# arkworks-rs/accumulation

Hardware: AMD Instinct MI355X
Metric: MSM throughput (point-scalar pairs/sec) at 2^20 Pallas (higher is better)
Workload: dtype u32; 1 GPU; 2^20-pair pallas MSM per GPU (north_star size; scalars uniform in [0, r), G_i = k_i*G), key resident + precomputed window multiples; pairs_per_gpu=1048576, curve=pallas, precomputed_key=True, parallelism=point-sharded x1, window_bits=20, pipeline=bucket-per-lane (k_prep_local_t + k_accum_bpl; skewed scalars re-run chunked), window_widths=9 x 20 + 4 x 19 bits = 256 (MsmGeom::n_narrow), msms_in_flight=3, full=False

## Files before the change

### accumulation_amd/csrc/api_pipeline.inc

```

#define HIP_TRY(expr)                                                                                  \
  do {                                                                                                 \
    hipError_t _e = (expr);                                                                            \
    if (_e != hipSuccess) {                                                                            \
      fprintf(stderr, "[amsm] HIP error %s (%d) at %s:%d: %s\n", hipGetErrorName(_e), (int)_e, __FILE__, \
              __LINE__, #expr);                                                                        \
      return _e == hipErrorOutOfMemory ? AMSM_E_OOM : AMSM_E_HIP;                                      \
    }                                                                                                  \
  } while (0)

#define TRY(expr)            \
  do {                       \
    int _s = (expr);         \
    if (_s != AMSM_OK) return _s; \
  } while (0)

int ensure(DevBuf& b, size_t bytes) {
  if (b.bytes >= bytes && b.p) return AMSM_OK;
  if (b.p) HIP_TRY(hipFree(b.p));
  b.p = nullptr;
  b.bytes = 0;
  size_t want = bytes + bytes / 8 + 256;
  HIP_TRY(hipMalloc(&b.p, want));
  b.bytes = want;
// ... 176 lines not shown
#define AMSM_DBG(name)                                    \
  do {                                                    \
    if (amsm_debug()) {                                   \
      fprintf(stderr, "[amsm] %s ...", name);             \
      hipError_t e_ = hipDeviceSynchronize();             \
      fprintf(stderr, " %s\n", hipGetErrorString(e_));    \
    }                                                     \
  } while (0)

int prep_fork(amsm_ctx* ctx) {
  HIP_TRY(hipEventRecord(ctx->fork, ctx->stream));
  HIP_TRY(hipStreamWaitEvent(ctx->s_prep, ctx->fork, 0));
  return AMSM_OK;
}

template <class Fq>
int bases_alt(amsm_ctx* ctx, const amsm_bases* b, const amsm_bases** out);

inline size_t bpl_min_pairs(const amsm_bases*) { return msel::P2(18) + 1; }

inline bool bpl_geom(amsm_ctx* ctx, const amsm_bases* bases, size_t base_off, size_t n, int group_shift, int c_plain, MsmGeom* out) {
  MsmGeom g;
  if (make_geom(ctx, bases, base_off, n, &g, group_shift, c_plain) != AMSM_OK) return false;
  if (g.groups == 1u && g.precomp) {
    u32 b = 1;
    while ((1ull << b) < n) b++;
    unsigned long long abs_max = (unsigned long long)g.base_off + n - 1ull + (unsigned long long)(g.W - 1u) * g.table_stride;
    unsigned long long rel_max = ((unsigned long long)(g.W - 1u) << b) | ((1ull << b) - 1ull);
    if (rel_max < abs_max) g.idx_rel_bits = b;
  }
  g.bpl = 1;
  {
    unsigned long long raw_max = 0;
    (void)top_window_shift_curve(ctx->curve, (int)g.c, (int)g.W, (int)g.n_narrow, &raw_max);
    unsigned long long top_reach = std::min<unsigned long long>(g.nb, raw_max << (g.top_shift + (g.n_narrow ? 1u : 0u)));
    top_reach = std::max<unsigned long long>(1024ull, top_reach);
    const unsigned long long per_win = ((unsigned long long)n * 1024ull + g.nb - 1) / g.nb;
    const unsigned long long per_top = ((unsigned long long)n * 1024ull + top_reach - 1) / top_reach;
    const unsigned long long wins = g.precomp ? g.W : 1ull;
    g.part_max = (u32)std::min<unsigned long long>(0xffffffffull, g.precomp ? (wins - 1ull) * per_win + per_top : std::max(per_win, per_top));
    if (g.groups > 1u) g.part_max = (g.part_max + 1u) / 2u;
  }
  g.red_s = std::min<u32>(32u, g.nb);
  g.red_threads = g.nb / g.red_s;
  if (!prep_bpl_supported(g)) return false;
  *out = g;
  return true;
}

inline bool bps_geom(amsm_ctx* ctx, const amsm_bases* bases, size_t base_off, size_t n, int group_shift, MsmGeom* out) {
  MsmGeom g;
  if (make_geom(ctx, bases, base_off, n, &g, group_shift) != AMSM_OK) return false;
  if (g.groups == 1u) {
// ... 18 lines not shown
inline bool red2_applies(const amsm_ctx*, const MsmGeom& g) { return g.nb >= (1u << 18) && (g.nb & 1023u) == 0u; }
template <class Fq>
int msm_plan(amsm_ctx* ctx, Slot* sl, const amsm_bases* bases, size_t base_off, size_t n, int group_shift, bool* short_prep_out,
             const amsm_bases** eff = nullptr, bool force_chunked = false) {
  const bool quad = true;
  MsmGeom g;
  const size_t rec = xyzz_bytes<Fq>();
  const msel::Choice ch = choose_pipeline(ctx, bases, n, group_shift, force_chunked);
  auto common = [&]() -> int {
    u32 red_blocks = cdiv(g.red_threads * (quad ? 4u : 1u), 256);
    if (red2_applies(ctx, g)) {
      TRY(ensure(sl->red2_rc, (size_t)g.n_sets * (g.nb / 1024u + 1024u) * rec));
      red_blocks = std::max(red_blocks, cdiv((g.nb / 1024u + 1024u) * 4u, 256) + 1u);
    }
    TRY(ensure(sl->buckets, (size_t)g.B * rec));
    TRY(ensure(sl->red_out, (size_t)g.n_sets * red_blocks * rec));
    TRY(ensure(sl->fold_out, (size_t)g.n_sets * rec + 64));
    TRY(ensure_pinned(sl, g.n_sets * rec + 64));
    return ensure_red_ticket(ctx, sl, g.n_sets);
  };
  if (ch.pipeline == msel::BUCKET_PER_LANE && bpl_geom(ctx, bases, base_off, n, group_shift, ch.plain_window, &g)) {
    sl->geom = g;
    if (eff) *eff = bases;
    TRY(ensure(sl->vals_a, prep_bpl_part_entries(g) * 8 + 64));
    TRY(ensure(sl->vals_b, (size_t)prep_bpl_partitions(g) * prep_bpl_stride(g) * 4 + 64));
    TRY(ensure(sl->bpl_grp, (size_t)prep_bpl_partitions(g) * prep_bpl_groups_per_partition() * 8 + 64));
    TRY(ensure(sl->bpl_order, (size_t)prep_bpl_partitions(g) * prep_bpl_groups_per_partition() * 64 * 4 + 64));
    TRY(common());
    TRY(ensure(sl->prep_small, 64 + prep_small_words(g) * sizeof(u32) + 256));
    *short_prep_out = true;
    return AMSM_OK;
  }
  if (bases->bpl) TRY(bases_alt<Fq>(ctx, bases, &bases));
  if (eff) *eff = bases;
  if (ch.pipeline == msel::BUCKET_SPLIT && bps_geom(ctx, bases, base_off, n, group_shift, &g)) {
    sl->geom = g;
    const u32 P = prep_bps_partitions(g, g.bps_log2_l);
    TRY(ensure(sl->vals_a, prep_bps_part_entries(g, g.bps_log2_l) * 4 + 64));
    TRY(ensure(sl->vals_b, (size_t)P * prep_bps_stride(g, g.bps_log2_l) * 4 + 64));
    TRY(ensure(sl->bpl_grp, (size_t)P * 16 * 8 + 64));
    TRY(ensure(sl->bpl_order, (size_t)g.B * 4 + 64));
    TRY(common());
    TRY(ensure(sl->prep_small, 64 + prep_small_words(g) * sizeof(u32) + 256));
    *short_prep_out = true;
    return AMSM_OK;
  }
  TRY(make_geom(ctx, bases, base_off, n, &g, group_shift));
// ... 1125 lines not shown
```

### accumulation_amd/csrc/kern_fr.hip

```cpp
#include "launch.h"
#include "vec_kernels.h"
#include "prep_kernels.h"

#include <algorithm>
#include <cmath>
#include <atomic>
#include <cstdlib>
#include <cstring>

namespace amsm {

static inline u32 cdiv_(u32 a, u32 b) { return (a + b - 1) / b; }
static u32 stream_grid(u32 n) {
  constexpr u32 per_cu = 64;
  static const u32 cus = [] {
    int dev = 0;
    hipDeviceProp_t prop;
    if (hipGetDevice(&dev) != hipSuccess || hipGetDeviceProperties(&prop, dev) != hipSuccess) return 256u;
    return (u32)std::max(1, prop.multiProcessorCount);
  }();
  return std::max(1u, std::min(cdiv_(n, 256), cus * per_cu));
}

void launch_bounds(hipStream_t st, const void* keys_sorted, bool keys16, u32* vals_sorted, MsmGeom g, u32* start,
// ... 5 lines not shown
    hipLaunchKernelGGL((k_bounds<u32>), dim3(cdiv_(g.B, 256)), dim3(256), 0, st, (const u32*)keys_sorted, vals_sorted,
                       g, start, items);
}

constexpr u32 PREP_MAX_P = 4096;
static PrepGeom prep_geom(const MsmGeom& g) {
  PrepGeom pg;
  pg.SH = 4;
  while (((g.B + (1u << pg.SH) - 1u) >> pg.SH) > 512u && pg.SH < 10u) pg.SH++;
  while (((g.B + (1u << pg.SH) - 1u) >> pg.SH) > PREP_MAX_P) pg.SH++;
  pg.P = (g.B + (1u << pg.SH) - 1u) >> pg.SH;
  pg.SPB = g.S <= 16u ? 512u : 256u;
  unsigned long long max_idx = (unsigned long long)g.base_off + g.n - 1ull +
                               (g.precomp ? (unsigned long long)(g.W - 1u) * g.table_stride : 0ull);
  if (g.idx_rel_bits) max_idx = ((unsigned long long)(g.W - 1u) << g.idx_rel_bits) | ((1ull << g.idx_rel_bits) - 1ull);
  pg.IB = 1;
  while ((max_idx >> pg.IB) != 0ull) pg.IB++;
  while (pg.IB + pg.SH > 31u && pg.SH > 0u && ((g.B + (1u << (pg.SH - 1)) - 1u) >> (pg.SH - 1)) <= PREP_MAX_P) pg.SH--;
  pg.P = (g.B + (1u << pg.SH) - 1u) >> pg.SH;
  const u32 budget_words = 37888u, fixed_words = 2u * (1u << pg.SH) + 1024u;
  pg.CAP = budget_words > fixed_words + 4096u ? budget_words - fixed_words : 0u;
  pg.HEAVY = std::max<u32>(4u * (g.E / pg.P + 1u), 1u << 17);
  pg.FIX = 0;
  return pg;
}
static size_t prep_heavy_words(const MsmGeom& g) { return (size_t)g.B + 4096 + 64; }
size_t prep_small_words(const MsmGeom& g) { return 4 * (PREP_MAX_P + 1) + 1 + 3 * prep_heavy_words(g) + PREP_MAX_HEAVY; }
static size_t prep_local_lds(const PrepGeom& pg) { return (2 * (size_t)(1u << pg.SH) + 1024 + pg.CAP) * sizeof(u32); }
constexpr size_t PREP_LDS_LIMIT = 160 * 1024;
static std::atomic<unsigned long long> prep_local_attr_devices{0};
static void prep_local_attr() {
  int dev = 0;
  if (hipGetDevice(&dev) != hipSuccess || dev < 0 || dev >= 64) dev = 63;
  const unsigned long long bit = 1ull << dev;
  if (dev != 63 && (prep_local_attr_devices.load(std::memory_order_acquire) & bit)) return;
  (void)hipFuncSetAttribute((const void*)k_prep_local, hipFuncAttributeMaxDynamicSharedMemorySize, 152 * 1024);
  prep_local_attr_devices.fetch_or(bit, std::memory_order_release);
}
static size_t prep_scatter_lds(const MsmGeom& g, const PrepGeom& pg) {
  const size_t cap = (size_t)pg.SPB * g.S;
  return (3 * (size_t)pg.P + cap) * sizeof(u32) + cap * sizeof(uint16_t);
}
bool prep_supported(const MsmGeom& g) {
  if (g.n == 0 || g.S > 32u) return false;
  PrepGeom pg = prep_geom(g);
  return pg.SH <= 12u && pg.IB + pg.SH <= 31u && prep_scatter_lds(g, pg) <= PREP_LDS_LIMIT &&
         prep_local_lds(pg) <= PREP_LDS_LIMIT && (pg.P + 256) * sizeof(u32) <= 64 * 1024;
}

constexpr u32 BPL_LOCAL_FIXED_WORDS = 3u * BPL_NB + 2u * BPL_BINS + 2u * BPL_GROUPS + 2u;
constexpr u32 BPL_LOCAL_BUDGET_WORDS = 40960u;
static PrepGeom prep_bpl_geom(const MsmGeom& g) {
  PrepGeom pg;
  pg.SH = 10;
  pg.P = g.B >> pg.SH;
  pg.SPB = g.S <= 16u ? 512u : 256u;
  unsigned long long max_idx = (unsigned long long)g.base_off + g.n - 1ull +
                               (g.precomp ? (unsigned long long)(g.W - 1u) * g.table_stride : 0ull);
  if (g.idx_rel_bits) max_idx = ((unsigned long long)(g.W - 1u) << g.idx_rel_bits) | ((1ull << g.idx_rel_bits) - 1ull);
  pg.IB = 1;
  while ((max_idx >> pg.IB) != 0ull) pg.IB++;
  pg.CAP = BPL_LOCAL_BUDGET_WORDS - BPL_LOCAL_FIXED_WORDS;
  pg.HEAVY = 0xffffffffu;
  const unsigned long long per = std::max<unsigned long long>(((unsigned long long)g.E + pg.P - 1) / std::max(1u, pg.P), g.part_max);
  pg.FIX = (u32)std::min<unsigned long long>(pg.CAP, (per + per / 4ull + 2048ull + 15ull) & ~15ull);
  return pg;
}
size_t prep_bpl_part_entries(const MsmGeom& g) {
  PrepGeom pg = prep_bpl_geom(g);
  return std::max<size_t>(g.E, pg.FIX ? (size_t)pg.P * pg.FIX : 0);
}
static size_t prep_bpl_local_lds(const PrepGeom& pg) { return (size_t)(BPL_LOCAL_FIXED_WORDS + pg.CAP) * sizeof(u32); }
static size_t prep_bpl_scatter_lds(const MsmGeom& g, const PrepGeom& pg) {
  const size_t cap = (size_t)pg.SPB * g.S;
  return (3 * (size_t)pg.P + 2 * cap) * sizeof(u32) + cap * sizeof(uint16_t);
}
u32 prep_bpl_partitions(const MsmGeom& g) { return g.B >> 10; }
u32 prep_bpl_groups_per_partition() { return BPL_GROUPS; }
u32 prep_bpl_stride(const MsmGeom& g) {
  const u32 P = std::max(1u, prep_bpl_partitions(g));
  const unsigned long long per = std::max<unsigned long long>(((unsigned long long)g.E + P - 1) / P, g.part_max);
  return (u32)((per + per / 4ull + 4096ull + 1023ull) & ~1023ull);
}
bool prep_bpl_supported(const MsmGeom& g) {
  if (g.S > 32u || g.n == 0 || g.n_sets != g.groups * sets_per_group(g)) return false;
  if (g.B < (1u << 16) || (g.B & 1023u) || (g.B >> 10) > PREP_MAX_P || ((g.B >> 10) & 3u)) return false;
  PrepGeom pg = prep_bpl_geom(g);
  if (pg.IB > 30u) return false;
  if ((unsigned long long)g.E / pg.P + 1024ull > pg.CAP) return false;
  if (g.part_max && (unsigned long long)g.part_max + 5ull * (unsigned long long)std::sqrt((double)g.part_max) > pg.CAP) return false;
  return prep_bpl_scatter_lds(g, pg) <= PREP_LDS_LIMIT && prep_bpl_local_lds(pg) <= PREP_LDS_LIMIT &&
         (unsigned long long)pg.P * prep_bpl_stride(g) < (1ull << 31);
}
static std::atomic<unsigned long long> prep_bpl_attr_devices{0};
template <class KS>
static void prep_bpl_attr(KS scatter_kernel) {
  int dev = 0;
  if (hipGetDevice(&dev) != hipSuccess || dev < 0 || dev >= 64) dev = 63;
  const unsigned long long bit = 1ull << dev;
  (void)hipFuncSetAttribute((const void*)scatter_kernel, hipFuncAttributeMaxDynamicSharedMemorySize, (int)PREP_LDS_LIMIT);
  if (dev != 63 && (prep_bpl_attr_devices.load(std::memory_order_acquire) & bit)) return;
  static_assert((BPL_LOCAL_BUDGET_WORDS) * sizeof(u32) <= PREP_LDS_LIMIT, "k_prep_local_t's LDS must fit a workgroup");
  (void)hipFuncSetAttribute((const void*)k_prep_local_t, hipFuncAttributeMaxDynamicSharedMemorySize, (int)PREP_LDS_LIMIT);
  prep_bpl_attr_devices.fetch_or(bit, std::memory_order_release);
}

constexpr u32 bps_local_fixed_words(u32 nbp) { return 4u * nbp + 1024u + BPL_BINS + 2u * BPS_GROUPS + 2u; }
constexpr u32 BPS_LOCAL_BUDGET_WORDS = 37888u;
static PrepGeom prep_bps_geom(const MsmGeom& g, u32 log2_l) {
  PrepGeom pg;
  pg.SH = 10u - log2_l;
  pg.P = g.B >> pg.SH;
  pg.SPB = g.S <= 16u ? 512u : 256u;
  unsigned long long max_idx = (unsigned long long)g.base_off + g.n - 1ull +
                               (g.precomp ? (unsigned long long)(g.W - 1u) * g.table_stride : 0ull);
  if (g.idx_rel_bits) max_idx = ((unsigned long long)(g.W - 1u) << g.idx_rel_bits) | ((1ull << g.idx_rel_bits) - 1ull);
  pg.IB = 1;
  while ((max_idx >> pg.IB) != 0ull) pg.IB++;
  pg.CAP = BPS_LOCAL_BUDGET_WORDS - bps_local_fixed_words(1u << pg.SH);
  pg.HEAVY = 0xffffffffu;
  const unsigned long long per = ((unsigned long long)g.E + pg.P - 1) / std::max(1u, pg.P);
  pg.FIX = (u32)std::min<unsigned long long>(pg.CAP, (per + per / 2ull + 1024ull + 15ull) & ~15ull);
  return pg;
}
size_t prep_bps_part_entries(const MsmGeom& g, u32 log2_l) {
  PrepGeom pg = prep_bps_geom(g, log2_l);
  return std::max<size_t>(g.E, pg.FIX ? (size_t)pg.P * pg.FIX : 0);
}
static size_t prep_bps_local_lds(const PrepGeom& pg) {
  return (size_t)(bps_local_fixed_words(1u << pg.SH) + pg.CAP) * sizeof(u32);
}
u32 prep_bps_partitions(const MsmGeom& g, u32 log2_l) { return g.B >> (10u - log2_l); }
u32 prep_bps_stride(const MsmGeom& g, u32 log2_l) {
  const u32 P = std::max(1u, prep_bps_partitions(g, log2_l));
  const unsigned long long per = ((unsigned long long)g.E + P - 1) / P;
  return (u32)((per + per / 2ull + 4096ull + 1023ull) & ~1023ull);
}
int prep_bps_choose(const MsmGeom& g) {
  if (!g.precomp || g.n == 0 || g.S > 32u || g.B < 64u || (g.B & (g.B - 1u))) return -1;
  unsigned long long want = 128;
  while (want * 24576ull < g.E) want <<= 1;
  for (int l = 0; l <= 6; l++) {
    if ((10 - l) < 0 || (g.B >> (10 - l)) == 0) continue;
    const unsigned long long P = g.B >> (10 - l);
    if (P < want && l < 6) continue;
// ... 125 lines not shown
    }                                                                                                                \
    const size_t lds_scatter = prep_scatter_lds(g, pg);                                                              \
    if (g.S <= 16u) {                                                                                                \
      if (lds_scatter > 64 * 1024)                                                                                   \
        (void)hipFuncSetAttribute((const void*)k_prep_scatter<FR, 16, 1>, hipFuncAttributeMaxDynamicSharedMemorySize, \
                                  (int)PREP_LDS_LIMIT);                                                              \
      hipLaunchKernelGGL((k_prep_scatter<FR, 16, 1>), dim3(cdiv_(g.n, pg.SPB)), dim3(512), lds_scatter, st, scalars, \
                         mont, g, pg, part_start, part_cursor, b.part, b.err);                                       \
    } else {                                                                                                         \
      if (lds_scatter > 64 * 1024)                                                                                   \
        (void)hipFuncSetAttribute((const void*)k_prep_scatter<FR, 32, 1>, hipFuncAttributeMaxDynamicSharedMemorySize, \
                                  (int)PREP_LDS_LIMIT);                                                              \
      hipLaunchKernelGGL((k_prep_scatter<FR, 32, 1>), dim3(cdiv_(g.n, pg.SPB)), dim3(256), lds_scatter, st, scalars, \
                         mont, g, pg, part_start, part_cursor, b.part, b.err);                                       \
    }                                                                                                                \
    hipLaunchKernelGGL(k_prep_local_s, dim3(pg.P), dim3(1024), prep_bps_local_lds(pg), st,                           \
                       pg.FIX ? part_cursor : part_start, b.part, g, pg,                                             \
                       prep_bps_stride(g, log2_l), log2_l, b.ents_t, (BplGroup*)b.grp, b.order, b.err);              \
    return 0;                                                                                                        \
  }                                                                                                                  \
  template <>                                                                                                        \
  int launch_prep_bpl<FR>(hipStream_t st, const u32* scalars, int mont, MsmGeom g, const PrepBplBuffers& b) {        \
    PrepGeom pg = prep_bpl_geom(g);                                                                                  \
    u32* part_total = b.d_small;                                                                                     \
    u32* part_start = b.d_small + (PREP_MAX_P + 1);                                                                  \
    u32* part_cursor = b.d_small + 2 * (PREP_MAX_P + 1);                                                             \
    PrepHeavy hv;                                                                                                    \
    hv.n = b.d_small + 4 * (PREP_MAX_P + 1);                                                                         \
    hv.cnt = hv.n + 1;                                                                                               \
    hv.ids = hv.cnt + 64;                                  \
    hv.cur = hv.end = hv.ids;                                                                                        \
    {                  \
      size_t zero_bytes = (16 + 4 * (PREP_MAX_P + 1) + 1) * sizeof(u32);                                             \
      zero_bytes = (zero_bytes + 255) & ~(size_t)255;                                                                \
      if (b.err != b.d_small - 16) return -1;                                                                        \
      if (hipMemsetAsync(b.err, 0, zero_bytes, st) != hipSuccess) return -1;                                         \
    }                                                                                                                \
    if (g.S <= 16u) prep_bpl_attr(k_prep_scatter<FR, 16, 1, true>);                                                  \
    else prep_bpl_attr(k_prep_scatter<FR, 32, 1, true>);                                                             \
    if (!pg.FIX) {                                                                                                   \
      PrepGeom ph = pg;                                                                                              \
      ph.SPB = 1024;                                                                                                 \
      hipLaunchKernelGGL((k_prep_hist<FR>), dim3(cdiv_(g.n, 1024)), dim3(1024), pg.P * sizeof(u32), st, scalars,      \
                         mont, g, ph, part_total, b.err);                                                            \
      hipLaunchKernelGGL(k_prep_scan, dim3(1), dim3(1024), 0, st, part_total, part_start, pg.P, pg.HEAVY, hv);       \
    }                                                                                                                \
    if (g.S <= 16u)                                                                                                  \
      hipLaunchKernelGGL((k_prep_scatter<FR, 16, 1, true>), dim3(cdiv_(g.n, pg.SPB)), dim3(512),                     \
                         prep_bpl_scatter_lds(g, pg), st, scalars, mont, g, pg, part_start, part_cursor, b.part, b.err); \
    else                                             \
      hipLaunchKernelGGL((k_prep_scatter<FR, 32, 1, true>), dim3(cdiv_(g.n, pg.SPB)), dim3(256),                     \
                         prep_bpl_scatter_lds(g, pg), st, scalars, mont, g, pg, part_start, part_cursor, b.part, b.err); \
    hipLaunchKernelGGL(k_prep_local_t, dim3(pg.P), dim3(1024), prep_bpl_local_lds(pg), st,                           \
                       pg.FIX ? part_cursor : part_start, (const u64*)b.part, g, pg, prep_bpl_stride(g), b.ents_t,   \
                       (BplGroup*)b.grp, b.order, b.err);                                                            \
    return 0;                                                                                                        \
  }                                                                                                                  \
  template <>                                                                                                        \
  void launch_digits<FR>(hipStream_t st, const u32* scalars, int mont, MsmGeom g, void* keys, bool keys16, u32* vals, \
                         u32* err) {                                                                                 \
    if (keys16)                                                                                                      \
      hipLaunchKernelGGL((k_digits<FR, uint16_t>), dim3(cdiv_(g.n, 256)), dim3(256), 0, st, scalars, mont, g,         \
                         (uint16_t*)keys, vals, err);                                                                \
    else                                                                                                             \
      hipLaunchKernelGGL((k_digits<FR, u32>), dim3(cdiv_(g.n, 256)), dim3(256), 0, st, scalars, mont, g, (u32*)keys,  \
                         vals, err);                                                                                 \
  }                                                                                                                  \
  template <>                                                                                                        \
  void launch_skew_probe<FR>(hipStream_t st, const u32* scalars, int mont, u32 n, DigitWalk walk, u32* d_flag,       \
                             const u32* d_tv_words) {                                                               \
    hipLaunchKernelGGL((k_skew_probe<FR>), dim3(1), dim3(1024), 0, st, scalars, mont, n, walk, d_flag, d_tv_words);  \
  }                                                                                                                  \
  template <>                                                                                                        \
  void launch_vec_random<FR>(hipStream_t st, u32* out, u64 seed, u32 n, int mont) {                                  \
    hipLaunchKernelGGL((k_vec_random<FR>), dim3(cdiv_(n, 256)), dim3(256), 0, st, out, seed, n, mont);               \
  }                                                                                                                  \
  template <>                                                                                                        \
  void launch_vec_hadamard<FR>(hipStream_t st, const u32* a, const u32* b, u32* out, u32 n) {                        \
// ... 102 lines not shown
```

### accumulation_amd/csrc/msm_types.h

```cpp
#pragma once
#include <stdint.h>

#include "blake2s.h"

namespace amsm {

typedef uint32_t u32;
typedef uint64_t u64;

struct SampleConsts {
  b2s::SamplePrefix prefix;
  u32 b[12];
  u32 r2[12];
  u32 root[12];
  u32 half[12];
  u32 exp[12];
  u32 exp_bits;
  u32 two_adicity;
  u32 cofactor[4];
  u32 cofactor_bits;
};
enum { SAMPLE_CNT_PENDING = 0, SAMPLE_CNT_EXHAUSTED = 1, SAMPLE_CNT_IDENTITY = 2, SAMPLE_CNT_WORDS = 3 };

struct PointsCheckConsts {
// ... 57 lines not shown
  u32 skip_ones;
};
AMSM_GEOM_FN DigitWalk digit_walk_of(const MsmGeom& g) {
  DigitWalk d;
  d.c = g.c;
  d.W = g.W;
  d.n_narrow = g.n_narrow;
  d.top_shift = g.top_shift;
  d.skip_ones = g.skip_ones;
  return d;
}
AMSM_GEOM_FN u32 narrow_windows_for(u32 c) {
  const u32 W = 255u / c + 1u, nn = W * c - 256u;
  return nn < W ? nn : ~0u;
}
AMSM_GEOM_FN u32 sets_per_group(const MsmGeom& g) { return g.precomp ? 1u : g.W + g.top_split; }
AMSM_GEOM_FN u32 window_set(const MsmGeom& g, u32 w, u32 i) {
  const u32 sb = (g.groups > 1u && g.group_shift == 0u) ? 1u : 0u;
  return g.precomp ? 0u : w + ((g.top_split && w == g.W - 1u) ? ((i >> sb) & 1u) : 0u);
}
AMSM_GEOM_FN u32 entry_abs_index(const MsmGeom& g, u32 v) {
  return g.idx_rel_bits ? (g.base_off + (v & ((1u << g.idx_rel_bits) - 1u)) + (v >> g.idx_rel_bits) * g.table_stride) : v;
}
AMSM_GEOM_FN u32 chunk_of(const MsmGeom& g, u32 pos) { return pos < g.T0 ? pos / g.K0 : g.nA + (pos - g.T0) / g.K0b; }
AMSM_GEOM_FN u32 chunk_start(const MsmGeom& g, u32 c) { return c < g.nA ? c * g.K0 : g.T0 + (c - g.nA) * g.K0b; }

struct CombineArgs {
  const u32* vec[VEC_MAX];
  u32 len[VEC_MAX];
  u32 coeff[VEC_MAX][8];
  const u32* hiding;
  u32 hiding_len;
  u32 n_vecs;
  u32 n;
};

constexpr int POLY_MAX = 8;
constexpr u32 POLY_LOG_E = 2, POLY_E = 1u << POLY_LOG_E, POLY_T = 256u * POLY_E;
struct PolyArgs {
  const u32* c[POLY_MAX];
  u32* q[POLY_MAX];
  u32 len[POLY_MAX];
  u32 off[POLY_MAX];
  u32 z[POLY_MAX][8];
  u32 pw[POLY_MAX][8][8];
  u32 zt[8];
// ... 26 lines not shown
```

### accumulation_amd/csrc/prep_kernels.h

```cpp
#pragma once
#include "fp.h"
#include "msm_types.h"
#include "vec_kernels.h"

namespace amsm {

struct PrepGeom {
  u32 SH;
  u32 P;
  u32 SPB;
  u32 IB;
  u32 CAP;
  u32 HEAVY;
  u32 FIX;
};

constexpr u32 PREP_HEAVY_SLICES = 64, PREP_HEAVY_GRID = 1024, PREP_MAX_HEAVY = 4096;
struct PrepHeavy {
  u32* n;
  u32* ids;
  u32* cnt;
  u32* cur;
  u32* end;
};

constexpr u32 PREP_ENTRY_LAST = 0x40000000u;

AMSM_DEV u32 lds_count(u32* ctr, u32 idx) {
  const u64 active = __ballot(1);
  const u32 first = __builtin_amdgcn_readfirstlane(idx);
  const u64 same = __ballot(idx == first);
  if (same == active) {
    const u32 lane = __lane_id();
    const u32 below = (u32)__popcll(same & ((1ull << lane) - 1ull));
    u32 base = 0;
    if (below == 0) base = atomicAdd(&ctr[first], (u32)__popcll(same));
    base = __builtin_amdgcn_readfirstlane(base);
// ... 75 lines not shown
  for (u32 d = 1; d < T; d <<= 1) {
    u32 v = t >= d ? lds[t - d] : 0u;
    __syncthreads();
    lds[t] += v;
    __syncthreads();
  }
  u32 run = lds[t] - sum;
  for (u32 k = lo; k < hi; k++) {
    u32 v = in[k];
    out[k] = run;
    run += v;
  }
  if (with_total && t == T - 1) out[n] = lds[T - 1];
}

__global__ void __launch_bounds__(1024)
    k_prep_scan(const u32* __restrict__ part_total, u32* __restrict__ part_start, u32 P, u32 heavy_min, PrepHeavy hv) {
  __shared__ u32 lds[1024];
  block_exclusive_scan(part_total, part_start, P, true, lds);
  for (u32 p = threadIdx.x; p < P; p += blockDim.x)
    if (part_total[p] > heavy_min) hv.ids[atomicAdd(hv.n, 1u)] = p;
}

template <class Fr, int MAXW, int SPT, bool WIDE = false>
__global__ void __launch_bounds__(512)
    k_prep_scatter(const u32* __restrict__ scalars, int mont, MsmGeom g, PrepGeom pg, const u32* __restrict__ part_start,
                   u32* __restrict__ part_cursor, u32* __restrict__ part, u32* __restrict__ err = nullptr) {
  extern __shared__ u32 prep_lds[];
  const u32 cap = pg.SPB * g.S;
  u32* cnt = prep_lds;
  u32* loff = prep_lds + pg.P;
  u32* gbase = prep_lds + 2 * pg.P;
  u32* staged = prep_lds + 3 * pg.P;
  uint16_t* staged_p = reinterpret_cast<uint16_t*>(staged + (WIDE ? 2u : 1u) * cap);
  const u32 t = threadIdx.x, T = blockDim.x;
  for (u32 p = t; p < pg.P; p += T) cnt[p] = 0;
  __syncthreads();
  u32 rk[SPT][MAXW / 2];
  Fe<Fr> sreg[SPT];
#pragma unroll
  for (int r = 0; r < SPT; r++) {
#pragma unroll
    for (int k = 0; k < MAXW / 2; k++) rk[r][k] = 0;
    u32 i = blockIdx.x * pg.SPB + r * T + t;
    if (i < g.n) {
      sreg[r] = fe_load<Fr>(scalars + (size_t)i * 8);
      if (g.skip_ones) fe_drop_stored_one<Fr>(sreg[r], mont);
      if (mont) sreg[r] = fe_from_mont<Fr>(sreg[r]);
      const u32 bad = scalar_entries_unrolled_reg<Fr, MAXW>(sreg[r], g, i, [&](int w, u32 key, u32) {
        u32 rank = atomicAdd(&cnt[key >> pg.SH], 1u);
        rk[r][w >> 1] |= rank << ((w & 1) * 16);
      });
      if (pg.FIX && bad && err) atomicOr(err, 1u);
    }
  }
  __syncthreads();
  constexpr u32 RSV_MAX = 4;
  u32 rsv[RSV_MAX], rsv_base[RSV_MAX];
// ... 1 lines not shown
  u32 lo = min(t * per, pg.P), hi = min(lo + per, pg.P);
  {
    u32* sl = reinterpret_cast<u32*>(staged);
    u32 sum = 0;
    for (u32 p = lo; p < hi; p++) sum += cnt[p];
    sl[t] = sum;
    __syncthreads();
    for (u32 d = 1; d < T; d <<= 1) {
      u32 v = t >= d ? sl[t - d] : 0u;
      __syncthreads();
      sl[t] += v;
      __syncthreads();
    }
    u32 run = sl[t] - sum;
#pragma unroll
    for (u32 q = 0; q < RSV_MAX; q++) {
      u32 p = lo + q;
      rsv[q] = 0;
      rsv_base[q] = 0;
      if (p < hi) {
        u32 v = cnt[p];
        loff[p] = run;
        if (v) {
          rsv_base[q] = pg.FIX ? p * pg.FIX : part_start[p];
          rsv[q] = atomicAdd(&part_cursor[p], v);
        }
        run += v;
      }
    }
    for (u32 p = lo + RSV_MAX; p < hi; p++) {
      u32 v = cnt[p];
      loff[p] = run;
      gbase[p] = v ? (pg.FIX ? p * pg.FIX : part_start[p]) + atomicAdd(&part_cursor[p], v) : 0u;
      run += v;
    }
  }
  __syncthreads();
  const u32 low = (1u << pg.SH) - 1u;
#pragma unroll
  for (int r = 0; r < SPT; r++) {
    u32 i = blockIdx.x * pg.SPB + r * T + t;
    if (i < g.n)
      scalar_entries_unrolled_reg<Fr, MAXW>(sreg[r], g, i, [&](int w, u32 key, u32 val) {
        u32 p = key >> pg.SH;
        u32 rank = (rk[r][w >> 1] >> ((w & 1) * 16)) & 0xffffu;
        u32 slot = loff[p] + rank;
        if (WIDE) reinterpret_cast<u64*>(staged)[slot] = ((u64)(key & low) << 32) | val;
        else staged[slot] = (val & 0x80000000u) | ((key & low) << pg.IB) | (val & 0x7fffffffu);
        staged_p[slot] = (uint16_t)p;
      });
  }
#pragma unroll
  for (u32 q = 0; q < RSV_MAX; q++)
    if (lo + q < hi) gbase[lo + q] = rsv_base[q] + rsv[q];
  __syncthreads();
  u32 total = loff[pg.P - 1] + cnt[pg.P - 1];
  for (u32 j = t; j < total; j += T) {
    u32 p = staged_p[j];
    const u32 dst = gbase[p] + (j - loff[p]);
    if (pg.FIX && dst - p * pg.FIX >= pg.FIX) continue;
    if (WIDE) reinterpret_cast<u64*>(part)[dst] = reinterpret_cast<const u64*>(staged)[j];
    else part[dst] = staged[j];
  }
}

__global__ void __launch_bounds__(1024)
    k_prep_local(const u32* __restrict__ part_start, const u32* __restrict__ part, MsmGeom g, PrepGeom pg,
                 u32* __restrict__ vals_sorted, u32* __restrict__ start, u32* __restrict__ items, u32* __restrict__ item_off,
                 u32* __restrict__ part_items, PrepHeavy hv) {
  extern __shared__ u32 prep_lds[];
  const u32 NB = 1u << pg.SH;
  u32* cnt = prep_lds;
  u32* off = prep_lds + NB;
  u32* sl = prep_lds + 2 * NB;
  const u32 p = blockIdx.x, t = threadIdx.x, T = blockDim.x;
  const u32 ps = part_start[p], pe = part_start[p + 1];
  const u32 low = NB - 1u, idx_mask = (1u << pg.IB) - 1u;
  const bool heavy = (pe - ps) > pg.HEAVY;
  for (u32 k = t; k < NB; k += T) cnt[k] = heavy ? hv.cnt[(p << pg.SH) + k] : 0u;
  __syncthreads();
  const u32 body_lo = min((ps + 3u) & ~3u, pe), body_hi = max(body_lo, pe & ~3u);
  const bool skew = (pe - ps) > 4u * (g.E / pg.P + 1u);
  auto count = [&](u32 e) {
    u32 k = (e >> pg.IB) & low;
    if (skew) lds_count(cnt, k);
// ... 199 lines not shown
constexpr u32 BPL_ENTRY_PAD = 0x40000000u;
constexpr u32 BPL_BINS = 256;
constexpr u32 BPL_SPLIT = 64;
constexpr u32 BPL_NB = 1024;
constexpr u32 BPL_LANES = BPL_NB + BPL_SPLIT;
constexpr u32 BPL_GROUPS = BPL_LANES / BPL_GROUP;
struct BplGroup {
  u32 base;
  u32 m;
};
AMSM_DEV void bpl_slot(u32 s, u32& pos, u32& half) {
  if (s < BPL_SPLIT) {
    pos = s >> 1;
    half = 1u + (s & 1u);
  } else if (s >= BPL_NB) {
    pos = BPL_SPLIT / 2u + ((s - BPL_NB) >> 1);
    half = 1u + (s & 1u);
  } else {
    pos = s;
    half = 0u;
  }
}

__global__ void __launch_bounds__(1024)
    k_prep_local_t(const u32* __restrict__ part_start, const u64* __restrict__ part, MsmGeom g, PrepGeom pg, u32 stride,
                   u32* __restrict__ ents_t, BplGroup* __restrict__ grp, u32* __restrict__ order, u32* __restrict__ err) {
  extern __shared__ u32 prep_lds[];
  const u32 NB = BPL_NB, NG = BPL_GROUPS;
  u32* cnt = prep_lds;
  u32* cur = cnt + NB;
  u32* ord = cur + NB;
  u32* bins = ord + NB;
  u32* bscan = bins + BPL_BINS;
  u32* gm = bscan + BPL_BINS;
  u32* gb = gm + NG;
  u32* stage = gb + NG + 1;
  u32* sl = stage;
  const u32 p = blockIdx.x, t = threadIdx.x, T = blockDim.x;
  const u32 ps = pg.FIX ? p * pg.FIX : part_start[p];
  const u32 n_p = pg.FIX ? part_start[p] : part_start[p + 1] - ps;
  const u32 pe = ps + (pg.FIX ? min(n_p, pg.FIX) : n_p);
  const u32 low = NB - 1u, idx_mask = (1u << pg.IB) - 1u, b0 = p << pg.SH;
  const bool fits = n_p <= pg.CAP && (!pg.FIX || n_p <= pg.FIX);
  for (u32 k = t; k < NB; k += T) cnt[k] = 0;
  for (u32 k = t; k < BPL_BINS; k += T) bins[k] = 0;
  for (u32 k = t; k < NG; k += T) gm[k] = 0;
  __syncthreads();
  if (fits)
    for (u32 j = ps + t; j < pe; j += T) atomicAdd(&cnt[(u32)(part[j] >> 32) & low], 1u);
  __syncthreads();
  const u32 c_t = t < NB ? cnt[t] : 0u;
  sl[t] = c_t;
  __syncthreads();
  for (u32 d = 1; d < T; d <<= 1) {
    u32 v = t >= d ? sl[t - d] : 0u;
    __syncthreads();
    sl[t] += v;
    __syncthreads();
  }
  if (t < NB) cur[t] = sl[t] - c_t;
  const u32 bin = min(c_t, BPL_BINS - 1u);
  u32 rank = 0;
  if (t < NB) rank = atomicAdd(&bins[bin], 1u);
  __syncthreads();
  if (fits)
    for (u32 j = ps + t; j < pe; j += T) {
      const u64 e = part[j];
      const u32 k = (u32)(e >> 32) & low, lo = (u32)e;
      const u32 pos = atomicAdd(&cur[k], 1u);
      stage[pos] = (lo & 0x80000000u) | entry_abs_index(g, lo & idx_mask);
    }
  if (t < BPL_BINS) bscan[t] = bins[BPL_BINS - 1u - t];
  __syncthreads();
  for (u32 d = 1; d < BPL_BINS; d <<= 1) {
    u32 v = (t < BPL_BINS && t >= d) ? bscan[t - d] : 0u;
    __syncthreads();
    if (t < BPL_BINS) bscan[t] += v;
    __syncthreads();
  }
  if (t < BPL_BINS) bins[BPL_BINS - 1u - t] = bscan[t] - bins[BPL_BINS - 1u - t];
  __syncthreads();
  u32 my_pos = 0;
  if (t < NB) {
    my_pos = bins[bin] + rank;
    ord[my_pos] = t;
    const u32 h0 = (c_t + 1u) >> 1;
    if (my_pos < BPL_SPLIT / 2u) atomicMax(&gm[0], h0);
    else if (my_pos < BPL_SPLIT) atomicMax(&gm[NG - 1u], h0);
    else atomicMax(&gm[my_pos / BPL_GROUP], c_t);
  }
  __syncthreads();
  if (t == 0) {
    u32 run = 0;
    for (u32 q = 0; q < NG; q++) {
      gb[q] = run;
      run += gm[q] * BPL_GROUP;
    }
    gb[NG] = run;
  }
  __syncthreads();
  const u32 total = gb[NG];
  const bool ok = fits && total <= stride;
  if (!ok && t == 0) atomicOr(err + 1, 1u);
  if (t < NG) {
    BplGroup h;
    h.base = p * stride + gb[t];
    h.m = ok ? gm[t] : 0u;
    grp[p * NG + t] = h;
  }
  if (t < NB) {
    u32* o = order + (size_t)p * BPL_LANES;
    if (my_pos < BPL_SPLIT / 2u) o[2u * my_pos] = o[2u * my_pos + 1u] = b0 + t;
    else if (my_pos < BPL_SPLIT) o[BPL_NB + 2u * (my_pos - BPL_SPLIT / 2u)] = o[BPL_NB + 2u * (my_pos - BPL_SPLIT / 2u) + 1u] = b0 + t;
    else o[my_pos] = b0 + t;
  }
  if (!ok) return;
  for (u32 j = t; j < total; j += T) {
    u32 q = 0;
    while (q + 1u < NG && gb[q + 1u] <= j) q++;
    const u32 k = (j - gb[q]) / BPL_GROUP, l = j % BPL_GROUP;
    u32 pos, half;
    bpl_slot(q * BPL_GROUP + l, pos, half);
    const u32 kb = ord[pos], c = cnt[kb], h0 = (c + 1u) >> 1;
    const u32 off = half == 2u ? h0 : 0u, sz = half == 0u ? c : (half == 1u ? h0 : c - h0);
    ents_t[(size_t)p * stride + j] = k < sz ? stage[cur[kb] - c + off + k] : BPL_ENTRY_PAD;
  }
}

constexpr u32 BPS_LANES = 1024, BPS_GROUPS = BPS_LANES / BPL_GROUP;
__global__ void __launch_bounds__(1024)
    k_prep_local_s(const u32* __restrict__ part_start, const u32* __restrict__ part, MsmGeom g, PrepGeom pg, u32 stride,
                   u32 log2_l, u32* __restrict__ ents_t, BplGroup* __restrict__ grp, u32* __restrict__ order,
                   u32* __restrict__ err) {
  extern __shared__ u32 prep_lds[];
  const u32 NBP = 1u << pg.SH, L = 1u << log2_l, NG = BPS_GROUPS;
  u32* cnt = prep_lds;
  u32* cur = cnt + NBP;
  u32* beg = cur + NBP;
  u32* ord = beg + NBP;
  u32* sl = ord + NBP;
// ... 88 lines not shown
```

Measured before the change: 967.5 million pairs/s.

## Pack bucket-per-lane prep entries into 32 bits with per-slice scalar cursors

Replaces the 64-bit (bucket, index) partition entries of the bucket-per-lane prep with 32-bit packed words holding sign, low bucket bits, window and the low bits of the scalar index. The high index bits become an implicit sub-slice, so each partition gets NSUB fixed-size slices with their own cursors. This removes the histogram and scan kernels and halves scatter staging and partition traffic. In exchange, the local kernel must walk the slice cursors serially per thread to locate entries, and more padding is reserved per slice.

After: 973.7 million pairs/s (median of 6 runs). No clear change (+0.6%).

```diff
diff --git a/accumulation_amd/csrc/api_pipeline.inc b/accumulation_amd/csrc/api_pipeline.inc
--- a/accumulation_amd/csrc/api_pipeline.inc
+++ b/accumulation_amd/csrc/api_pipeline.inc
@@ -222,13 +222,6 @@
 inline bool bpl_geom(amsm_ctx* ctx, const amsm_bases* bases, size_t base_off, size_t n, int group_shift, int c_plain, MsmGeom* out) {
   MsmGeom g;
   if (make_geom(ctx, bases, base_off, n, &g, group_shift, c_plain) != AMSM_OK) return false;
-  if (g.groups == 1u && g.precomp) {
-    u32 b = 1;
-    while ((1ull << b) < n) b++;
-    unsigned long long abs_max = (unsigned long long)g.base_off + n - 1ull + (unsigned long long)(g.W - 1u) * g.table_stride;
-    unsigned long long rel_max = ((unsigned long long)(g.W - 1u) << b) | ((1ull << b) - 1ull);
-    if (rel_max < abs_max) g.idx_rel_bits = b;
-  }
   g.bpl = 1;
   {
     unsigned long long raw_max = 0;
@@ -293,7 +286,7 @@
   if (ch.pipeline == msel::BUCKET_PER_LANE && bpl_geom(ctx, bases, base_off, n, group_shift, ch.plain_window, &g)) {
     sl->geom = g;
     if (eff) *eff = bases;
-    TRY(ensure(sl->vals_a, prep_bpl_part_entries(g) * 8 + 64));
+    TRY(ensure(sl->vals_a, prep_bpl_part_entries(g) * 4 + 64));
     TRY(ensure(sl->vals_b, (size_t)prep_bpl_partitions(g) * prep_bpl_stride(g) * 4 + 64));
     TRY(ensure(sl->bpl_grp, (size_t)prep_bpl_partitions(g) * prep_bpl_groups_per_partition() * 8 + 64));
     TRY(ensure(sl->bpl_order, (size_t)prep_bpl_partitions(g) * prep_bpl_groups_per_partition() * 64 * 4 + 64));
diff --git a/accumulation_amd/csrc/kern_fr.hip b/accumulation_amd/csrc/kern_fr.hip
--- a/accumulation_amd/csrc/kern_fr.hip
+++ b/accumulation_amd/csrc/kern_fr.hip
@@ -51,10 +51,14 @@
   pg.CAP = budget_words > fixed_words + 4096u ? budget_words - fixed_words : 0u;
   pg.HEAVY = std::max<u32>(4u * (g.E / pg.P + 1u), 1u << 17);
   pg.FIX = 0;
+  pg.pk = BplPack{0, 0, 0};
   return pg;
 }
 static size_t prep_heavy_words(const MsmGeom& g) { return (size_t)g.B + 4096 + 64; }
-size_t prep_small_words(const MsmGeom& g) { return 4 * (PREP_MAX_P + 1) + 1 + 3 * prep_heavy_words(g) + PREP_MAX_HEAVY; }
+size_t prep_small_words(const MsmGeom& g) {
+  static_assert(BPL_MAX_CURSORS <= 4 * (PREP_MAX_P + 1), "the slice cursors of the bucket-per-lane prep fit the block's fixed part");
+  return 4 * (PREP_MAX_P + 1) + 1 + 3 * prep_heavy_words(g) + PREP_MAX_HEAVY;
+}
 static size_t prep_local_lds(const PrepGeom& pg) { return (2 * (size_t)(1u << pg.SH) + 1024 + pg.CAP) * sizeof(u32); }
 constexpr size_t PREP_LDS_LIMIT = 160 * 1024;
 static std::atomic<unsigned long long> prep_local_attr_devices{0};
@@ -77,32 +81,26 @@
          prep_local_lds(pg) <= PREP_LDS_LIMIT && (pg.P + 256) * sizeof(u32) <= 64 * 1024;
 }
 
-constexpr u32 BPL_LOCAL_FIXED_WORDS = 3u * BPL_NB + 2u * BPL_BINS + 2u * BPL_GROUPS + 2u;
-constexpr u32 BPL_LOCAL_BUDGET_WORDS = 40960u;
 static PrepGeom prep_bpl_geom(const MsmGeom& g) {
   PrepGeom pg;
-  pg.SH = 10;
+  pg.SH = BPL_SH;
   pg.P = g.B >> pg.SH;
   pg.SPB = g.S <= 16u ? 512u : 256u;
-  unsigned long long max_idx = (unsigned long long)g.base_off + g.n - 1ull +
-                               (g.precomp ? (unsigned long long)(g.W - 1u) * g.table_stride : 0ull);
-  if (g.idx_rel_bits) max_idx = ((unsigned long long)(g.W - 1u) << g.idx_rel_bits) | ((1ull << g.idx_rel_bits) - 1ull);
-  pg.IB = 1;
-  while ((max_idx >> pg.IB) != 0ull) pg.IB++;
-  pg.CAP = BPL_LOCAL_BUDGET_WORDS - BPL_LOCAL_FIXED_WORDS;
+  pg.IB = 0;
+  pg.CAP = BPL_LOCAL_CAP;
   pg.HEAVY = 0xffffffffu;
-  const unsigned long long per = std::max<unsigned long long>(((unsigned long long)g.E + pg.P - 1) / std::max(1u, pg.P), g.part_max);
-  pg.FIX = (u32)std::min<unsigned long long>(pg.CAP, (per + per / 4ull + 2048ull + 15ull) & ~15ull);
+  pg.pk = bpl_pack_geom(g);
+  pg.FIX = bpl_fixsub(g, pg.pk, pg.CAP);
   return pg;
 }
 size_t prep_bpl_part_entries(const MsmGeom& g) {
   PrepGeom pg = prep_bpl_geom(g);
-  return std::max<size_t>(g.E, pg.FIX ? (size_t)pg.P * pg.FIX : 0);
+  return (size_t)pg.P * pg.pk.NSUB * pg.FIX;
 }
 static size_t prep_bpl_local_lds(const PrepGeom& pg) { return (size_t)(BPL_LOCAL_FIXED_WORDS + pg.CAP) * sizeof(u32); }
 static size_t prep_bpl_scatter_lds(const MsmGeom& g, const PrepGeom& pg) {
   const size_t cap = (size_t)pg.SPB * g.S;
-  return (3 * (size_t)pg.P + 2 * cap) * sizeof(u32) + cap * sizeof(uint16_t);
+  return (3 * (size_t)pg.P + cap) * sizeof(u32) + cap * sizeof(uint16_t);
 }
 u32 prep_bpl_partitions(const MsmGeom& g) { return g.B >> 10; }
 u32 prep_bpl_groups_per_partition() { return BPL_GROUPS; }
@@ -115,7 +113,9 @@
   if (g.S > 32u || g.n == 0 || g.n_sets != g.groups * sets_per_group(g)) return false;
   if (g.B < (1u << 16) || (g.B & 1023u) || (g.B >> 10) > PREP_MAX_P || ((g.B >> 10) & 3u)) return false;
   PrepGeom pg = prep_bpl_geom(g);
-  if (pg.IB > 30u) return false;
+  if (1u + BPL_SH + pg.pk.WB + pg.pk.IL > 32u || ((1u << pg.pk.IL) % pg.SPB) != 0u) return false;
+  if (pg.pk.NSUB > BPL_MAX_NSUB || bpl_cursor_words(g, pg.pk) > BPL_MAX_CURSORS) return false;
+  if ((unsigned long long)prep_bpl_part_entries(g) >= (1ull << 31)) return false;
   if ((unsigned long long)g.E / pg.P + 1024ull > pg.CAP) return false;
   if (g.part_max && (unsigned long long)g.part_max + 5ull * (unsigned long long)std::sqrt((double)g.part_max) > pg.CAP) return false;
   return prep_bpl_scatter_lds(g, pg) <= PREP_LDS_LIMIT && prep_bpl_local_lds(pg) <= PREP_LDS_LIMIT &&
@@ -150,6 +150,7 @@
   pg.HEAVY = 0xffffffffu;
   const unsigned long long per = ((unsigned long long)g.E + pg.P - 1) / std::max(1u, pg.P);
   pg.FIX = (u32)std::min<unsigned long long>(pg.CAP, (per + per / 2ull + 1024ull + 15ull) & ~15ull);
+  pg.pk = BplPack{0, 0, 0};
   return pg;
 }
 size_t prep_bps_part_entries(const MsmGeom& g, u32 log2_l) {
@@ -321,38 +322,25 @@
   template <>                                                                                                        \
   int launch_prep_bpl<FR>(hipStream_t st, const u32* scalars, int mont, MsmGeom g, const PrepBplBuffers& b) {        \
     PrepGeom pg = prep_bpl_geom(g);                                                                                  \
-    u32* part_total = b.d_small;                                                                                     \
-    u32* part_start = b.d_small + (PREP_MAX_P + 1);                                                                  \
-    u32* part_cursor = b.d_small + 2 * (PREP_MAX_P + 1);                                                             \
-    PrepHeavy hv;                                                                                                    \
-    hv.n = b.d_small + 4 * (PREP_MAX_P + 1);                                                                         \
-    hv.cnt = hv.n + 1;                                                                                               \
-    hv.ids = hv.cnt + 64;                                  \
-    hv.cur = hv.end = hv.ids;                                                                                        \
-    {                  \
-      size_t zero_bytes = (16 + 4 * (PREP_MAX_P + 1) + 1) * sizeof(u32);                                             \
+    u32* slice_cursor = b.d_small;                 \
+    {                       \
+      size_t zero_bytes = (16 + (size_t)bpl_cursor_words(g, pg.pk)) * sizeof(u32);                                   \
       zero_bytes = (zero_bytes + 255) & ~(size_t)255;                                                                \
       if (b.err != b.d_small - 16) return -1;                                                                        \
       if (hipMemsetAsync(b.err, 0, zero_bytes, st) != hipSuccess) return -1;                                         \
     }                                                                                                                \
     if (g.S <= 16u) prep_bpl_attr(k_prep_scatter<FR, 16, 1, true>);                                                  \
     else prep_bpl_attr(k_prep_scatter<FR, 32, 1, true>);                                                             \
-    if (!pg.FIX) {                                                                                                   \
-      PrepGeom ph = pg;                                                                                              \
-      ph.SPB = 1024;                                                                                                 \
-      hipLaunchKernelGGL((k_prep_hist<FR>), dim3(cdiv_(g.n, 1024)), dim3(1024), pg.P * sizeof(u32), st, scalars,      \
-                         mont, g, ph, part_total, b.err);                                                            \
-      hipLaunchKernelGGL(k_prep_scan, dim3(1), dim3(1024), 0, st, part_total, part_start, pg.P, pg.HEAVY, hv);       \
-    }                                                                                                                \
     if (g.S <= 16u)                                                                                                  \
       hipLaunchKernelGGL((k_prep_scatter<FR, 16, 1, true>), dim3(cdiv_(g.n, pg.SPB)), dim3(512),                     \
-                         prep_bpl_scatter_lds(g, pg), st, scalars, mont, g, pg, part_start, part_cursor, b.part, b.err); \
+                         prep_bpl_scatter_lds(g, pg), st, scalars, mont, g, pg, (const u32*)nullptr, slice_cursor, b.part, \
+                         b.err);                                                                                      \
     else                                             \
       hipLaunchKernelGGL((k_prep_scatter<FR, 32, 1, true>), dim3(cdiv_(g.n, pg.SPB)), dim3(256),                     \
-                         prep_bpl_scatter_lds(g, pg), st, scalars, mont, g, pg, part_start, part_cursor, b.part, b.err); \
-    hipLaunchKernelGGL(k_prep_local_t, dim3(pg.P), dim3(1024), prep_bpl_local_lds(pg), st,                           \
-                       pg.FIX ? part_cursor : part_start, (const u64*)b.part, g, pg, prep_bpl_stride(g), b.ents_t,   \
-                       (BplGroup*)b.grp, b.order, b.err);                                                            \
+                         prep_bpl_scatter_lds(g, pg), st, scalars, mont, g, pg, (const u32*)nullptr, slice_cursor, b.part, \
+                         b.err);                                                                                      \
+    hipLaunchKernelGGL(k_prep_local_t, dim3(pg.P), dim3(BPL_LOCAL_T), prep_bpl_local_lds(pg), st, slice_cursor,      \
+                       b.part, g, pg, prep_bpl_stride(g), b.ents_t, (BplGroup*)b.grp, b.order, b.err);               \
     return 0;                                                                                                        \
   }                                                                                                                  \
   template <>                                                                                                        \
diff --git a/accumulation_amd/csrc/msm_types.h b/accumulation_amd/csrc/msm_types.h
--- a/accumulation_amd/csrc/msm_types.h
+++ b/accumulation_amd/csrc/msm_types.h
@@ -103,6 +103,53 @@
 AMSM_GEOM_FN u32 entry_abs_index(const MsmGeom& g, u32 v) {
   return g.idx_rel_bits ? (g.base_off + (v & ((1u << g.idx_rel_bits) - 1u)) + (v >> g.idx_rel_bits) * g.table_stride) : v;
 }
+
+constexpr u32 BPL_SH = 10;
+constexpr u32 BPL_MAX_CURSORS = 16384;
+constexpr u32 BPL_MAX_NSUB = 1024;
+struct BplPack {
+  u32 WB;
+  u32 IL;
+  u32 NSUB;
+};
+AMSM_GEOM_FN BplPack bpl_pack_geom(const MsmGeom& g) {
+  BplPack k;
+  k.WB = 0;
+  if (g.precomp)
+    while ((1u << k.WB) < g.W) k.WB++;
+  k.IL = 31u - BPL_SH - k.WB;
+  k.NSUB = (u32)(((u64)g.n + (1ull << k.IL) - 1ull) >> k.IL);
+  return k;
+}
+AMSM_GEOM_FN u32 bpl_pack(const BplPack& k, u32 neg, u32 bucket_low, u32 w, u32 i) {
+  return (neg << 31) | (bucket_low << (k.WB + k.IL)) | (k.WB ? (w << k.IL) : 0u) | (i & ((1u << k.IL) - 1u));
+}
+AMSM_GEOM_FN u32 bpl_sub_of(const BplPack& k, u32 i) { return i >> k.IL; }
+AMSM_GEOM_FN u32 bpl_entry_bucket(const BplPack& k, u32 e) { return (e >> (k.WB + k.IL)) & ((1u << BPL_SH) - 1u); }
+AMSM_GEOM_FN u32 bpl_entry_window(const BplPack& k, u32 e) { return k.WB ? ((e >> k.IL) & ((1u << k.WB) - 1u)) : 0u; }
+AMSM_GEOM_FN u32 bpl_entry_scalar(const BplPack& k, u32 sub, u32 e) { return (sub << k.IL) | (e & ((1u << k.IL) - 1u)); }
+AMSM_GEOM_FN u32 bpl_entry_table_word(const MsmGeom& g, const BplPack& k, u32 sub, u32 e) {
+  return (e & 0x80000000u) | (g.base_off + bpl_entry_scalar(k, sub, e) + (g.precomp ? bpl_entry_window(k, e) * g.table_stride : 0u));
+}
+AMSM_GEOM_FN u32 bpl_ceil_sqrt(u64 x) {
+  u32 s = 0;
+  while ((u64)s * s < x) s++;
+  return s;
+}
+AMSM_GEOM_FN u32 bpl_sub_expect(const MsmGeom& g, const BplPack& k) {
+  const u32 P = g.B >> BPL_SH;
+  u64 per = P ? ((u64)g.E + P - 1u) / P : 0ull;
+  if (per < g.part_max) per = g.part_max;
+  const u64 full = (u64)g.n < (1ull << k.IL) ? (u64)g.n : (1ull << k.IL);
+  return g.n ? (u32)((per * full + g.n - 1u) / g.n) : 0u;
+}
+AMSM_GEOM_FN u32 bpl_fixsub(const MsmGeom& g, const BplPack& k, u32 cap) {
+  const u64 e = bpl_sub_expect(g, k);
+  const u64 fix = (e + e / 4ull + 6ull * bpl_ceil_sqrt(e) + 512ull + 15ull) & ~15ull;
+  return (u32)(fix < cap ? fix : cap);
+}
+AMSM_GEOM_FN u64 bpl_cursor_words(const MsmGeom& g, const BplPack& k) { return (u64)(g.B >> BPL_SH) * k.NSUB; }
+
 AMSM_GEOM_FN u32 chunk_of(const MsmGeom& g, u32 pos) { return pos < g.T0 ? pos / g.K0 : g.nA + (pos - g.T0) / g.K0b; }
 AMSM_GEOM_FN u32 chunk_start(const MsmGeom& g, u32 c) { return c < g.nA ? c * g.K0 : g.T0 + (c - g.nA) * g.K0b; }
 
diff --git a/accumulation_amd/csrc/prep_kernels.h b/accumulation_amd/csrc/prep_kernels.h
--- a/accumulation_amd/csrc/prep_kernels.h
+++ b/accumulation_amd/csrc/prep_kernels.h
@@ -13,6 +13,7 @@
   u32 CAP;
   u32 HEAVY;
   u32 FIX;
+  BplPack pk;
 };
 
 constexpr u32 PREP_HEAVY_SLICES = 64, PREP_HEAVY_GRID = 1024, PREP_MAX_HEAVY = 4096;
@@ -134,7 +135,7 @@
     if (part_total[p] > heavy_min) hv.ids[atomicAdd(hv.n, 1u)] = p;
 }
 
-template <class Fr, int MAXW, int SPT, bool WIDE = false>
+template <class Fr, int MAXW, int SPT, bool BPL = false>
 __global__ void __launch_bounds__(512)
     k_prep_scatter(const u32* __restrict__ scalars, int mont, MsmGeom g, PrepGeom pg, const u32* __restrict__ part_start,
                    u32* __restrict__ part_cursor, u32* __restrict__ part, u32* __restrict__ err = nullptr) {
@@ -144,8 +145,9 @@
   u32* loff = prep_lds + pg.P;
   u32* gbase = prep_lds + 2 * pg.P;
   u32* staged = prep_lds + 3 * pg.P;
-  uint16_t* staged_p = reinterpret_cast<uint16_t*>(staged + (WIDE ? 2u : 1u) * cap);
+  uint16_t* staged_p = reinterpret_cast<uint16_t*>(staged + cap);
   const u32 t = threadIdx.x, T = blockDim.x;
+  const u32 nsub = BPL ? pg.pk.NSUB : 1u, sub = BPL ? bpl_sub_of(pg.pk, blockIdx.x * pg.SPB) : 0u;
   for (u32 p = t; p < pg.P; p += T) cnt[p] = 0;
   __syncthreads();
   u32 rk[SPT][MAXW / 2];
@@ -193,8 +195,8 @@
         u32 v = cnt[p];
         loff[p] = run;
         if (v) {
-          rsv_base[q] = pg.FIX ? p * pg.FIX : part_start[p];
-          rsv[q] = atomicAdd(&part_cursor[p], v);
+          rsv_base[q] = pg.FIX ? (p * nsub + sub) * pg.FIX : part_start[p];
+          rsv[q] = atomicAdd(&part_cursor[p * nsub + sub], v);
         }
         run += v;
       }
@@ -202,7 +204,7 @@
     for (u32 p = lo + RSV_MAX; p < hi; p++) {
       u32 v = cnt[p];
       loff[p] = run;
-      gbase[p] = v ? (pg.FIX ? p * pg.FIX : part_start[p]) + atomicAdd(&part_cursor[p], v) : 0u;
+      gbase[p] = v ? (pg.FIX ? (p * nsub + sub) * pg.FIX : part_start[p]) + atomicAdd(&part_cursor[p * nsub + sub], v) : 0u;
       run += v;
     }
   }
@@ -216,7 +218,7 @@
         u32 p = key >> pg.SH;
         u32 rank = (rk[r][w >> 1] >> ((w & 1) * 16)) & 0xffffu;
         u32 slot = loff[p] + rank;
-        if (WIDE) reinterpret_cast<u64*>(staged)[slot] = ((u64)(key & low) << 32) | val;
+        if (BPL) staged[slot] = bpl_pack(pg.pk, val >> 31, key & low, (u32)w, i);
         else staged[slot] = (val & 0x80000000u) | ((key & low) << pg.IB) | (val & 0x7fffffffu);
         staged_p[slot] = (uint16_t)p;
       });
@@ -229,9 +231,8 @@
   for (u32 j = t; j < total; j += T) {
     u32 p = staged_p[j];
     const u32 dst = gbase[p] + (j - loff[p]);
-    if (pg.FIX && dst - p * pg.FIX >= pg.FIX) continue;
-    if (WIDE) reinterpret_cast<u64*>(part)[dst] = reinterpret_cast<const u64*>(staged)[j];
-    else part[dst] = staged[j];
+    if (pg.FIX && dst - (p * nsub + sub) * pg.FIX >= pg.FIX) continue;
+    part[dst] = staged[j];
   }
 }
 
@@ -477,8 +478,12 @@
   }
 }
 
-__global__ void __launch_bounds__(1024)
-    k_prep_local_t(const u32* __restrict__ part_start, const u64* __restrict__ part, MsmGeom g, PrepGeom pg, u32 stride,
+constexpr u32 BPL_LOCAL_FIXED_WORDS = 3u * BPL_NB + 2u * BPL_BINS + 2u * BPL_GROUPS + 2u;
+constexpr u32 BPL_LOCAL_BUDGET_WORDS = 40960u;
+constexpr u32 BPL_LOCAL_CAP = BPL_LOCAL_BUDGET_WORDS - BPL_LOCAL_FIXED_WORDS;
+constexpr u32 BPL_LOCAL_T = 1024;
+__global__ void __launch_bounds__(BPL_LOCAL_T)
+    k_prep_local_t(const u32* __restrict__ part_cursor, const u32* __restrict__ part, MsmGeom g, PrepGeom pg, u32 stride,
                    u32* __restrict__ ents_t, BplGroup* __restrict__ grp, u32* __restrict__ order, u32* __restrict__ err) {
   extern __shared__ u32 prep_lds[];
   const u32 NB = BPL_NB, NG = BPL_GROUPS;
@@ -491,18 +496,34 @@
   u32* gb = gm + NG;
   u32* stage = gb + NG + 1;
   u32* sl = stage;
+  u32* subc = ord;
   const u32 p = blockIdx.x, t = threadIdx.x, T = blockDim.x;
-  const u32 ps = pg.FIX ? p * pg.FIX : part_start[p];
-  const u32 n_p = pg.FIX ? part_start[p] : part_start[p + 1] - ps;
-  const u32 pe = ps + (pg.FIX ? min(n_p, pg.FIX) : n_p);
-  const u32 low = NB - 1u, idx_mask = (1u << pg.IB) - 1u, b0 = p << pg.SH;
-  const bool fits = n_p <= pg.CAP && (!pg.FIX || n_p <= pg.FIX);
+  const BplPack pk = pg.pk;
+  const u32 b0 = p << pg.SH, slice0 = p * pk.NSUB;
+  u32 total = 0;
+  bool fits = true;
+  for (u32 s = 0; s < pk.NSUB; s++) {
+    const u32 c = part_cursor[slice0 + s];
+    fits = fits && c <= pg.FIX;
+    total += min(c, pg.FIX);
+  }
+  fits = fits && total <= pg.CAP;
+  if (!fits) total = 0;
+  for (u32 s = t; s < pk.NSUB; s += T) subc[s] = min(part_cursor[slice0 + s], pg.FIX);
   for (u32 k = t; k < NB; k += T) cnt[k] = 0;
   for (u32 k = t; k < BPL_BINS; k += T) bins[k] = 0;
   for (u32 k = t; k < NG; k += T) gm[k] = 0;
   __syncthreads();
-  if (fits)
-    for (u32 j = ps + t; j < pe; j += T) atomicAdd(&cnt[(u32)(part[j] >> 32) & low], 1u);
+  u32 s = 0, s_lo = 0, s_hi = subc[0];
+  auto locate = [&](u32 j) {
+    while (j >= s_hi) {
+      s++;
+      s_lo = s_hi;
+      s_hi += subc[s];
+    }
+    return (slice0 + s) * pg.FIX + (j - s_lo);
+  };
+  for (u32 j = t; j < total; j += T) atomicAdd(&cnt[bpl_entry_bucket(pk, part[locate(j)])], 1u);
   __syncthreads();
   const u32 c_t = t < NB ? cnt[t] : 0u;
   sl[t] = c_t;
@@ -518,13 +539,12 @@
   u32 rank = 0;
   if (t < NB) rank = atomicAdd(&bins[bin], 1u);
   __syncthreads();
-  if (fits)
-    for (u32 j = ps + t; j < pe; j += T) {
-      const u64 e = part[j];
-      const u32 k = (u32)(e >> 32) & low, lo = (u32)e;
-      const u32 pos = atomicAdd(&cur[k], 1u);
-      stage[pos] = (lo & 0x80000000u) | entry_abs_index(g, lo & idx_mask);
-    }
+  s = 0, s_lo = 0, s_hi = subc[0];
+  for (u32 j = t; j < total; j += T) {
+    const u32 e = part[locate(j)];
+    const u32 pos = atomicAdd(&cur[bpl_entry_bucket(pk, e)], 1u);
+    stage[pos] = bpl_entry_table_word(g, pk, s, e);
+  }
   if (t < BPL_BINS) bscan[t] = bins[BPL_BINS - 1u - t];
   __syncthreads();
   for (u32 d = 1; d < BPL_BINS; d <<= 1) {
@@ -554,8 +574,8 @@
     gb[NG] = run;
   }
   __syncthreads();
-  const u32 total = gb[NG];
-  const bool ok = fits && total <= stride;
+  const u32 padded = gb[NG];
+  const bool ok = fits && padded <= stride;
   if (!ok && t == 0) atomicOr(err + 1, 1u);
   if (t < NG) {
     BplGroup h;
@@ -570,7 +590,7 @@
     else o[my_pos] = b0 + t;
   }
   if (!ok) return;
-  for (u32 j = t; j < total; j += T) {
+  for (u32 j = t; j < padded; j += T) {
     u32 q = 0;
     while (q + 1u < NG && gb[q + 1u] <= j) q++;
     const u32 k = (j - gb[q]) / BPL_GROUP, l = j % BPL_GROUP;
```
